# innnky/vispeech

Hardware: AMD Instinct MI355X
Metric: 44.1kHz samples/sec (higher is better)
Workload: dtype f32 (split-f16 MFMA, 3-term); 1 GPU; C3: 64 mixed zh/ja utterances (~5 s each) per GPU, 44.1 kHz, hop 512, phoneme/duration/F0/energy/noise supplied, random-init (synthetic) weights of configs/config.json; 2 batches in flight per GPU; utterances_per_gpu=64, global_batch=64, padded_frames=489, frames_padded=31296, frames_computed=28902, parallelism=shard1, generator=f16s, controls=all, batches_in_flight=2

## Files before the change

### vispeech_amd/csrc/conv_mfma.hip

```cpp
#include "kernels.h"

#include <cstdio>
#include <cstdlib>
#include <cstring>
#include <type_traits>

namespace vsp {

typedef float f32x16 __attribute__((ext_vector_type(16)));

size_t packed_conv_floats(int M, int Cin, int K) {
  const size_t mt = (M + 31) / 32, nc = (Cin + CONV_CK - 1) / CONV_CK;
  return mt * nc * (size_t)K * 1024;
}

void pack_conv_weights(float* dst, int M, int Cin, int K, const float* dense) {
  const int nc = (Cin + CONV_CK - 1) / CONV_CK;
  std::memset(dst, 0, packed_conv_floats(M, Cin, K) * sizeof(float));
  for (int row = 0; row < M; ++row) {
    const int mtile = row >> 5, rin = row & 31;
    for (int ci = 0; ci < Cin; ++ci) {
      const int chunk = ci / CONV_CK, cc = ci % CONV_CK;
      const int kk = cc >> 1, hh = cc & 1, lane = rin + 32 * hh, kg = kk >> 2, i = kk & 3;
      for (int tap = 0; tap < K; ++tap) {
        const size_t idx =
            (((((size_t)mtile * nc + chunk) * K + tap) * (CONV_CK / 8) + kg) * 64 + lane) * 4 + i;
        dst[idx] = dense[((size_t)row * Cin + ci) * K + tap];
      }
    }
  }
}

void pack_conv_weights_f16s(float* dst_f, int M, int Cin, int K, const float* dense) {
  const int nc = (Cin + CONV_CK - 1) / CONV_CK;
  std::memset(dst_f, 0, packed_conv_floats(M, Cin, K) * sizeof(float));
  uint16_t* dst = reinterpret_cast<uint16_t*>(dst_f);
  for (int row = 0; row < M; ++row) {
    const int mtile = row >> 5, rin = row & 31;
    for (int ci = 0; ci < Cin; ++ci) {
      const int chunk = ci / CONV_CK, cc = ci % CONV_CK;
      const int ks = cc >> 4, hh = (cc >> 3) & 1, j = cc & 7, lane = rin + 32 * hh;
      for (int tap = 0; tap < K; ++tap) {
        const float w = dense[((size_t)row * Cin + ci) * K + tap] * G16_WSCALE;
        const _Float16 h = (_Float16)w;
        const _Float16 l = (_Float16)(w - (float)h);
        const size_t blk = (((size_t)mtile * nc + chunk) * K + tap) * 2048;
        std::memcpy(dst + blk + ((size_t)(ks * 2 + 0) * 64 + lane) * 8 + j, &h, 2);
        std::memcpy(dst + blk + ((size_t)(ks * 2 + 1) * 64 + lane) * 8 + j, &l, 2);
      }
    }
  }
}

typedef _Float16 f16x8 __attribute__((ext_vector_type(8)));
typedef _Float16 f16x2 __attribute__((ext_vector_type(2)));
typedef unsigned u32x4 __attribute__((ext_vector_type(4)));

#ifndef CONV_DIAG
#define CONV_DIAG 0
#endif
#if CONV_DIAG & 1
#define CONV_MFMA16(a, b, c) ([&]() { asm volatile("" ::"v"(a), "v"(b)); return c; }())
#else
#define CONV_MFMA16(a, b, c) __builtin_amdgcn_mfma_f32_32x32x16_f16(a, b, c, 0, 0, 0)
#endif
#define CONV_RAW_BARRIER() asm volatile("s_waitcnt lgkmcnt(0)\n\ts_barrier" ::: "memory")
template <int N>
__device__ __forceinline__ void conv_vmcnt() {
  asm volatile("s_waitcnt vmcnt(%0)" ::"n"(N) : "memory");
}
constexpr int conv_ring_slots(int MT, int WM) { return 3; }

template <int MT, int NT>
struct ConvEpi {
  float bv[MT][16], cv[MT][16];
  unsigned rv[MT][NT][16], pv[MT][NT][16];
};
constexpr int CONV_OOR = 0x7ffffff0;

template <int MT, int NT, bool HOIST = true>
__device__ __forceinline__ void conv_epi_load(const ConvArgs& a, ConvEpi<MT, NT>& e, int mtile0, int n_mtiles, int t0, int wn,
                                              int l31, int h, int b, int what = 3) {
  const float* resb = a.res ? a.res + (size_t)b * a.r_bs : nullptr;
  float* outb = a.out + (size_t)b * a.o_bs;
  const float* condb = a.cond ? a.cond + (size_t)b * a.cond_bs : nullptr;
  const __amdgpu_buffer_rsrc_t ro = __builtin_amdgcn_make_buffer_rsrc(outb, 0, CONV_OOR, 0x00020000);
  const __amdgpu_buffer_rsrc_t rr = __builtin_amdgcn_make_buffer_rsrc(const_cast<float*>(resb ? resb : outb), 0, CONV_OOR, 0x00020000);
  const __amdgpu_buffer_rsrc_t ro2 = __builtin_amdgcn_make_buffer_rsrc(
      a.split_row ? a.out2 + (size_t)b * a.o2_bs : outb, 0, CONV_OOR, 0x00020000);
  auto row_vec = [&](const float* p, int row0, float* v) {
    v[0] = v[1] = v[2] = v[3] = 0.f;
    if (!p) return;
    if (row0 + 3 < a.M && (reinterpret_cast<uintptr_t>(p + row0) & 15) == 0) {
      const float4 t = *reinterpret_cast<const float4*>(p + row0);
      v[0] = t.x; v[1] = t.y; v[2] = t.z; v[3] = t.w;
    } else {
#pragma unroll
      for (int i = 0; i < 4; ++i)
        if (row0 + i < a.M) v[i] = p[row0 + i];
    }
  };
  const bool gate_ep = a.act == 2;
#pragma unroll
  for (int mt = 0; mt < MT; ++mt) {
    const int mtile = mtile0 + mt;
    if (what & 1) {
#pragma unroll
      for (int g = 0; g < 4; ++g) {
        row_vec(a.bias, mtile * 32 + 8 * g + 4 * h, &e.bv[mt][4 * g]);
        row_vec(condb, mtile * 32 + 8 * g + 4 * h, &e.cv[mt][4 * g]);
      }
    }
    if (!(what & 2)) continue;
    const bool second = a.split_row && mtile * 32 >= a.split_row;
    if constexpr (!HOIST) {
#pragma unroll
      for (int nt = 0; nt < NT; ++nt) {
        const int q = t0 + (wn * NT + nt) * 32 + l31;
        const bool qin = q < a.Nq && !gate_ep && mtile < n_mtiles;
#pragma unroll
        for (int r = 0; r < 16; ++r) {
          const int row = mtile * 32 + 8 * (r >> 2) + 4 * h + (r & 3);
          const bool st = qin && row < a.M;
          const int oo = st ? (row * (int)a.o_cs + q) * 4 : CONV_OOR;
// ... 309 lines not shown
    }
  }
  float v[16];
#pragma unroll
  for (int r = 0; r < 16; ++r) v[r] = tanhf(va[r]) * (1.f / (1.f + expf(-vb[r])));
  if (a.mask_post && !valid) {
#pragma unroll
    for (int r = 0; r < 16; ++r) v[r] = 0.f;
  }
#pragma unroll
  for (int r = 0; r < 16; ++r)
    __builtin_amdgcn_raw_buffer_store_b32(__float_as_uint(v[r]), ro, vo, (8 * (r >> 2) + (r & 3)) * ocs4, 0);
}

template <int S, int MT, int NT>
__device__ __forceinline__ void conv_store_slices(const ConvArgs& a, f32x16 (&acc)[MT][NT], int mtile0, int n_mtiles, int t0,
                                                  int wn, int l31, int h, int b, int len) {
#pragma unroll
  for (int ms = 0; ms < MT / S; ++ms)
#pragma unroll
    for (int nt = 0; nt < NT; ++nt) {
      const int tq = t0 + (wn * NT + nt) * 32;
      if constexpr (S == 1) {
        const int mtile = mtile0 + ms;
        if (mtile < n_mtiles && conv_tile_lean_ok(a, mtile)) {
          conv_tile_lean(a, acc[ms][nt], mtile, tq, l31, h, b, len);
          continue;
        }
      } else if constexpr (S == 2) {
        const int mtile = mtile0 + 2 * ms;
        if (conv_gate_lean_ok(a, mtile, n_mtiles)) {
          conv_gate_lean(a, acc[2 * ms][nt], acc[2 * ms + 1][nt], mtile, tq, l31, h, b, len);
          continue;
        }
      }
      f32x16 t[S][1];
#pragma unroll
      for (int u = 0; u < S; ++u) t[u][0] = acc[S * ms + u][nt];
      ConvEpi<S, 1> e;
      conv_epi_load<S, 1, false>(a, e, mtile0 + S * ms, n_mtiles, tq, 0, l31, h, b);
      conv_epi_store<S, 1>(a, t, e, mtile0 + S * ms, n_mtiles, tq, 0, l31, h, b, len);
    }
}
template <int MT, int NT>
__device__ __forceinline__ void conv_store_plain(const ConvArgs& a, f32x16 (&acc)[MT][NT], int mtile0, int n_mtiles, int t0,
                                                 int wn, int l31, int h, int b, int len) {
  if (a.act == 2) {
    if constexpr (MT % 2 == 0) conv_store_slices<2, MT, NT>(a, acc, mtile0, n_mtiles, t0, wn, l31, h, b, len);
  } else {
    conv_store_slices<1, MT, NT>(a, acc, mtile0, n_mtiles, t0, wn, l31, h, b, len);
  }
}

template <int MT, int NT, int WM, int WN, bool F16S, bool RING = false, bool PRUNE = false>
__global__ void __launch_bounds__(64 * WM * WN, F16S ? 2 : 1) conv1d_f32_mfma(ConvArgs a) {
  static_assert(!RING || F16S, "the weight ring serves the split-f16 path");
  static_assert(!PRUNE || (F16S && RING), "the pruned form is the split-f16 ring kernel");
  constexpr int BN = 32 * NT * WN;
  constexpr int LWP = BN + CONV_HALO;
  constexpr int NW = WM * WN;
  constexpr int KG = CONV_CK / 8;
  extern __shared__ __attribute__((aligned(16))) float xs[];
  constexpr int SB = MT * WM * 4096;
  constexpr int NS = conv_ring_slots(MT, WM), DEPTH = NS - 1;
  constexpr int PW = MT * WM * 4 / NW;
  static_assert(!RING || (MT * WM * 4) % NW == 0, "pieces divide over the waves");
  [[maybe_unused]] char* const ring = reinterpret_cast<char*>(xs) + (size_t)CONV_CK * LWP * sizeof(float);

  const int tid = threadIdx.x;
  const int wave = __builtin_amdgcn_readfirstlane(tid >> 6);
  const int lane = tid & 63;
  const int l31 = lane & 31, h = lane >> 5;
  const int wm = wave / WN, wn = wave % WN;
  const int b = blockIdx.z;
  const int t0 = blockIdx.x * BN;
  const int mtile0 = (blockIdx.y * WM + wm) * MT;
  const int n_mtiles = (a.M + 31) >> 5;
  const int len = a.lengths ? (int)a.lengths[b] : 0x7fffffff;
  const int LW = BN + (a.K - 1) * a.dil;
  const int total_it = a.nchunks * a.K;

  f32x16 acc[MT][NT];
#pragma unroll
  for (int mt = 0; mt < MT; ++mt)
#pragma unroll
    for (int nt = 0; nt < NT; ++nt)
#pragma unroll
      for (int r = 0; r < 16; ++r) {
        acc[mt][nt][r] = 0.f;
      }
  unsigned* const ph = reinterpret_cast<unsigned*>(xs);
  unsigned* const pl = ph + (CONV_CK / 2) * LWP;
  auto split_pair = [&](float x0, float x1, unsigned& whi, unsigned& wlo) { vsp_split_pair(x0, x1, whi, wlo); };

  const float4* wp4 = reinterpret_cast<const float4*>(a.wp);
  float4 a_cur[MT][KG], a_nxt[MT][KG];
  auto load_a = [&](int it, float4(&dst)[MT][KG]) {
#pragma unroll
    for (int mt = 0; mt < MT; ++mt) {
      const int mtile = mtile0 + mt;
      if (mtile < n_mtiles) {
        const float4* p = wp4 + (((size_t)mtile * total_it + it) * KG) * 64 + lane;
#pragma unroll
        for (int kg = 0; kg < KG; ++kg) dst[mt][kg] = p[kg * 64];
      } else {
#pragma unroll
        for (int kg = 0; kg < KG; ++kg) dst[mt][kg] = make_float4(0.f, 0.f, 0.f, 0.f);
      }
    }
  };
  if constexpr (!RING) load_a(0, a_cur);
  [[maybe_unused]] auto ring_dma = [&](int step) {
    char* dst = ring + (step % NS) * SB;
    if constexpr ((CONV_DIAG & 8) != 0) return;
#pragma unroll
    for (int u = 0; u < PW; ++u) {
      const int p = u * NW + wave;
      int mtile = blockIdx.y * (WM * MT) + (p >> 2);
      mtile = mtile < n_mtiles ? mtile : n_mtiles - 1;
      const float4* src = wp4 + (((size_t)mtile * total_it + step) * KG + (p & 3)) * 64 + lane;
      __builtin_amdgcn_global_load_lds((const __attribute__((address_space(1))) void*)src,
                                       (__attribute__((address_space(3))) void*)(dst + p * 1024), 16, 0, 0);
    }
  };
  constexpr bool PREF = RING && ((BN + CONV_HALO + 3) >> 2) <= 64;
  constexpr int RWPF = PREF ? (CONV_CK / 2) / NW : 1;
  constexpr int NPF = 2 * RWPF;
  [[maybe_unused]] int pf_step = -1000;
  [[maybe_unused]] auto ring_wait = [&](int step) {
    const int younger = total_it - 1 - step < DEPTH - 1 ? total_it - 1 - step : DEPTH - 1;
    const bool pf = PREF && step > pf_step && step - pf_step <= DEPTH;
    if (pf) {
      if (younger <= 0) conv_vmcnt<NPF>();
      else if (younger == 1) conv_vmcnt<PW + NPF>();
      else conv_vmcnt<2 * PW + NPF>();
    } else {
      if (younger <= 0) conv_vmcnt<0>();
      else if (younger == 1) conv_vmcnt<PW>();
      else conv_vmcnt<2 * PW>();
    }
  };
  static_assert(DEPTH <= 3, "ring_wait covers up to two younger steps");
  if constexpr (RING) {
#pragma unroll
    for (int d = 0; d < DEPTH; ++d)
      if (d < total_it) ring_dma(d);
  }

  const float* xb = a.x + (size_t)b * a.x_bs;
  const bool vec = ((a.x_cs & 3) == 0) && ((a.x_bs & 3) == 0) && ((reinterpret_cast<uintptr_t>(a.x) & 15) == 0);
  const int t_start = vec ? (((t0 - a.pad) >> 2) << 2) : (t0 - a.pad);
  const int off = (t0 - a.pad) - t_start;
  const int LW4 = (LW + off + 3) >> 2;
  const float* xsb = xs + h * LWP + wn * (NT * 32) + l31 + off;
  [[maybe_unused]] float4 pva[RWPF], pvb[RWPF];
  [[maybe_unused]] auto st_load = [&](int chunk) {
    const int t4 = t_start + 4 * lane;
    const bool tin = lane < LW4 && t4 >= 0 && t4 < a.T_in;
#pragma unroll
    for (int j = 0; j < RWPF; ++j) {
      const int ci = chunk * CONV_CK + 2 * (wave + j * NW);
      const float* pa = xb + (size_t)(tin && ci < a.Cin ? ci : 0) * a.x_cs + (tin ? t4 : 0);
      const float* pb = xb + (size_t)(tin && ci + 1 < a.Cin ? ci + 1 : 0) * a.x_cs + (tin ? t4 : 0);
      pva[j] = *reinterpret_cast<const float4*>(pa);
      pvb[j] = *reinterpret_cast<const float4*>(pb);
    }
  };
  typedef float f32x2v __attribute__((ext_vector_type(2)));
  [[maybe_unused]] const float slope_eff = a.in_act ? a.in_slope : 1.f;
  [[maybe_unused]] auto st_write = [&](int chunk) {
    if (lane >= LW4) return;
    const int t4 = t_start + 4 * lane;
    const bool tin = t4 >= 0 && t4 < a.T_in;
    const int lim = a.in_mask ? (len < a.T_in ? len : a.T_in) : a.T_in;
    const bool tfull = tin && t4 + 3 < lim;
#pragma unroll
    for (int j = 0; j < RWPF; ++j) {
      const int ci = chunk * CONV_CK + 2 * (wave + j * NW);
      const bool ina = tin && ci < a.Cin, inb = tin && ci + 1 < a.Cin;
      const float ea[4] = {pva[j].x, pva[j].y, pva[j].z, pva[j].w}, eb[4] = {pvb[j].x, pvb[j].y, pvb[j].z, pvb[j].w};
      unsigned wh4[4], wl4[4];
#pragma unroll
      for (int u = 0; u < 4; ++u) {
        f32x2v x = {ea[u], eb[u]};
        if (!(tfull && inb)) {
          x.x = (ina && t4 + u < lim) ? x.x : 0.f;
          x.y = (inb && t4 + u < lim) ? x.y : 0.f;
        }
        const f32x2v y = x * slope_eff;
        asm("v_max_f32 %0, %1, %2" : "=v"(x.x) : "v"(x.x), "v"(y.x));
        asm("v_max_f32 %0, %1, %2" : "=v"(x.y) : "v"(x.y), "v"(y.y));
        vsp_split_pair(x.x, x.y, wh4[u], wl4[u]);
      }
      const int o = (wave + j * NW) * LWP + 4 * lane;
      *reinterpret_cast<u32x4*>(ph + o) = u32x4{wh4[0], wh4[1], wh4[2], wh4[3]};
      *reinterpret_cast<u32x4*>(pl + o) = u32x4{wl4[0], wl4[1], wl4[2], wl4[3]};
    }
  };
  static_assert(!PRUNE || PREF, "the pruned form stages its window through the prefetch path");
  const bool pref = PRUNE || (PREF && vec && (CONV_DIAG & 2) == 0 && slope_eff >= 0.f && slope_eff <= 1.f);
  if constexpr (PREF) { if (pref) st_load(0); }
  int it = 0;
  for (int chunk = 0; chunk < a.nchunks; ++chunk) {
    if (pref) {
      if constexpr (PREF) st_write(chunk);
    } else if constexpr (PRUNE) {
    } else if (vec && F16S) {
      constexpr int RWP = (CONV_CK / 2) / NW;
      for (int q0 = 0; q0 < LW4; q0 += 64) {
        const int q4 = q0 + lane;
        const int t4 = t_start + 4 * q4;
        const bool tin = q4 < LW4 && t4 >= 0 && t4 < a.T_in;
        float4 va[RWP], vb[RWP];
#pragma unroll
        for (int j = 0; j < RWP; ++j) {
          const int ci = chunk * CONV_CK + 2 * (wave + j * NW);
          va[j] = vb[j] = make_float4(0.f, 0.f, 0.f, 0.f);
          if (tin && ci < a.Cin && !(CONV_DIAG & 2)) va[j] = *reinterpret_cast<const float4*>(xb + (size_t)ci * a.x_cs + t4);
          if (tin && ci + 1 < a.Cin && !(CONV_DIAG & 2)) vb[j] = *reinterpret_cast<const float4*>(xb + (size_t)(ci + 1) * a.x_cs + t4);
        }
        if (q4 < LW4) {
          const int lim = a.in_mask ? (len < a.T_in ? len : a.T_in) : a.T_in;
#pragma unroll
          for (int j = 0; j < RWP; ++j) {
            float ea[4] = {va[j].x, va[j].y, va[j].z, va[j].w}, eb[4] = {vb[j].x, vb[j].y, vb[j].z, vb[j].w};
            unsigned wh4[4], wl4[4];
#pragma unroll
            for (int u = 0; u < 4; ++u) {
              float x0 = (t4 + u < lim) ? ea[u] : 0.f, x1 = (t4 + u < lim) ? eb[u] : 0.f;
              if (a.in_act) { x0 = x0 > 0.f ? x0 : x0 * a.in_slope; x1 = x1 > 0.f ? x1 : x1 * a.in_slope; }
              split_pair(x0, x1, wh4[u], wl4[u]);
            }
            const int o = (wave + j * NW) * LWP + 4 * q4;
            *reinterpret_cast<u32x4*>(ph + o) = u32x4{wh4[0], wh4[1], wh4[2], wh4[3]};
            *reinterpret_cast<u32x4*>(pl + o) = u32x4{wl4[0], wl4[1], wl4[2], wl4[3]};
          }
        }
      }
    } else if (F16S) {
      for (int cp = wave; cp < CONV_CK / 2; cp += NW) {
        const int ci = chunk * CONV_CK + 2 * cp;
        const float* xr0 = xb + (size_t)ci * a.x_cs;
        const float* xr1 = xr0 + a.x_cs;
        for (int col = lane; col < LW; col += 64) {
          const int t = t0 - a.pad + col;
          float x0 = 0.f, x1 = 0.f;
          if (t >= 0 && t < a.T_in && !(a.in_mask && t >= len)) {
            if (ci < a.Cin) x0 = xr0[t];
            if (ci + 1 < a.Cin) x1 = xr1[t];
            if (a.in_act) { x0 = x0 > 0.f ? x0 : x0 * a.in_slope; x1 = x1 > 0.f ? x1 : x1 * a.in_slope; }
          }
          unsigned wh1, wl1;
          split_pair(x0, x1, wh1, wl1);
          ph[cp * LWP + col] = wh1;
          pl[cp * LWP + col] = wl1;
        }
      }
    } else if (vec) {
      constexpr int RW = CONV_CK / NW;
      for (int q0 = 0; q0 < LW4; q0 += 64) {
        const int q4 = q0 + lane;
        const int t4 = t_start + 4 * q4;
        const bool tin = q4 < LW4 && t4 >= 0 && t4 < a.T_in;
        float4 v[RW];
#pragma unroll
        for (int j = 0; j < RW; ++j) {
          const int ci = chunk * CONV_CK + wave + j * NW;
          v[j] = make_float4(0.f, 0.f, 0.f, 0.f);
          if (tin && ci < a.Cin) v[j] = *reinterpret_cast<const float4*>(xb + (size_t)ci * a.x_cs + t4);
        }
        if (q4 < LW4) {
          const int lim = a.in_mask ? (len < a.T_in ? len : a.T_in) : a.T_in;
#pragma unroll
          for (int j = 0; j < RW; ++j) {
            float e[4] = {v[j].x, v[j].y, v[j].z, v[j].w};
#pragma unroll
            for (int u = 0; u < 4; ++u) {
              float x = (t4 + u < lim) ? e[u] : 0.f;
              if (a.in_act) x = x > 0.f ? x : x * a.in_slope;
              e[u] = x;
            }
            *reinterpret_cast<float4*>(xs + (wave + j * NW) * LWP + 4 * q4) = make_float4(e[0], e[1], e[2], e[3]);
          }
        }
      }
    } else {
      for (int c = wave; c < CONV_CK; c += NW) {
        const int ci = chunk * CONV_CK + c;
        const bool cvalid = ci < a.Cin;
        const float* xr = xb + (size_t)ci * a.x_cs;
        float* dst = xs + c * LWP;
        for (int col = lane; col < LW; col += 64) {
          const int t = t0 - a.pad + col;
          float v = 0.f;
          if (cvalid && t >= 0 && t < a.T_in) {
            v = xr[t];
            if (a.in_mask && t >= len) v = 0.f;
            if (a.in_act) v = v > 0.f ? v : v * a.in_slope;
          }
          dst[col] = v;
        }
      }
    }
    if constexpr (!RING) __syncthreads();
    for (int tap = 0; tap < a.K; ++tap, ++it) {
      if constexpr (RING) {
        ring_wait(it);
        CONV_RAW_BARRIER();
        if (it + DEPTH < total_it) ring_dma(it + DEPTH);
        if constexpr (PREF) {
          if (pref && tap == 0 && chunk + 1 < a.nchunks) { st_load(chunk + 1); pf_step = it; }
        }
      } else {
        if (it + 1 < total_it) load_a(it + 1, a_nxt);
      }
      if constexpr (F16S) {
        const int col = wn * (NT * 32) + l31 + off + tap * a.dil;
#pragma unroll
        for (int ks = 0; ks < 2; ++ks) {
          f16x8 bh[NT], bl[NT];
#pragma unroll
          for (int nt = 0; nt < NT; ++nt) {
            const unsigned* p = ph + (8 * ks + 4 * h) * LWP + col + nt * 32;
            const unsigned* q = pl + (8 * ks + 4 * h) * LWP + col + nt * 32;
            bh[nt] = __builtin_bit_cast(f16x8, u32x4{p[0], p[LWP], p[2 * LWP], p[3 * LWP]});
            bl[nt] = __builtin_bit_cast(f16x8, u32x4{q[0], q[LWP], q[2 * LWP], q[3 * LWP]});
          }
#pragma unroll
          for (int mt = 0; mt < MT; ++mt) {
            f16x8 ah, al;
            if constexpr (RING) {
              const char* pa = ring + (it % NS) * SB + (wm * MT + mt) * 4096 + ks * 2048 + lane * 16;
              ah = *reinterpret_cast<const f16x8*>(pa);
              al = *reinterpret_cast<const f16x8*>(pa + 1024);
            } else {
              ah = __builtin_bit_cast(f16x8, a_cur[mt][2 * ks]);
              al = __builtin_bit_cast(f16x8, a_cur[mt][2 * ks + 1]);
            }
#pragma unroll
            for (int nt = 0; nt < NT; ++nt) acc[mt][nt] = CONV_MFMA16(ah, bh[nt], acc[mt][nt]);
#pragma unroll
            for (int nt = 0; nt < NT; ++nt) acc[mt][nt] = CONV_MFMA16(ah, bl[nt], acc[mt][nt]);
#pragma unroll
            for (int nt = 0; nt < NT; ++nt) acc[mt][nt] = CONV_MFMA16(al, bh[nt], acc[mt][nt]);
          }
        }
      }
      const float* xt = xsb + tap * a.dil;
#pragma unroll
      for (int kg = 0; kg < (F16S ? 0 : KG); ++kg) {
#pragma unroll
        for (int i = 0; i < 4; ++i) {
          const int kk = kg * 4 + i;
          float bv[NT];
#pragma unroll
          for (int nt = 0; nt < NT; ++nt) bv[nt] = xt[(2 * kk) * LWP + nt * 32];
#pragma unroll
          for (int mt = 0; mt < MT; ++mt) {
            const float av = i == 0 ? a_cur[mt][kg].x : i == 1 ? a_cur[mt][kg].y : i == 2 ? a_cur[mt][kg].z
                                                                                         : a_cur[mt][kg].w;
#pragma unroll
            for (int nt = 0; nt < NT; ++nt)
              acc[mt][nt] = __builtin_amdgcn_mfma_f32_32x32x2f32(av, bv[nt], acc[mt][nt], 0, 0, 0);
          }
        }
      }
      if constexpr (!RING) {
#pragma unroll
        for (int mt = 0; mt < MT; ++mt)
#pragma unroll
          for (int kg = 0; kg < KG; ++kg) a_cur[mt][kg] = a_nxt[mt][kg];
      }
    }
    if constexpr (RING) CONV_RAW_BARRIER();
    else __syncthreads();
  }

  if constexpr (F16S) {
#pragma unroll
    for (int mt = 0; mt < MT; ++mt)
#pragma unroll
      for (int nt = 0; nt < NT; ++nt)
#pragma unroll
        for (int r = 0; r < 16; ++r) acc[mt][nt][r] *= G16_UNSCALE;
  }
  if constexpr ((CONV_DIAG & 4) != 0) {
    float keep = 0.f;
#pragma unroll
    for (int mt = 0; mt < MT; ++mt)
#pragma unroll
      for (int nt = 0; nt < NT; ++nt) keep += acc[mt][nt][0];
    if (keep == 1.2345e-30f) a.out[0] = keep;
    return;
  }
  const float* resb = a.res ? a.res + (size_t)b * a.r_bs : nullptr;
  float* outb = a.out + (size_t)b * a.o_bs;
  const float* condb = a.cond ? a.cond + (size_t)b * a.cond_bs : nullptr;
  if (PRUNE || a.ups_s == 0) {
    conv_store_plain<MT, NT>(a, acc, mtile0, n_mtiles, t0, wn, l31, h, b, len);
    return;
  }
  if (a.act == 2) {
    if constexpr (MT % 2 == 0) {
#pragma unroll
      for (int mp = 0; mp < MT / 2; ++mp) {
        const int mtile = mtile0 + 2 * mp;
        if (mtile + 1 >= n_mtiles) continue;
#pragma unroll
        for (int nt = 0; nt < NT; ++nt) {
          const int q = t0 + (wn * NT + nt) * 32 + l31;
          if (q >= a.Nq) continue;
          const bool valid = q < len;
#pragma unroll
          for (int r = 0; r < 16; ++r) {
            const int rin = (r & 3) + 8 * (r >> 2) + 4 * h;
            const int ra = mtile * 32 + rin, rb = ra + 32;
            float va = acc[2 * mp][nt][r], vb = acc[2 * mp + 1][nt][r];
            if (a.bias) { va += a.bias[ra]; vb += a.bias[rb]; }
// ... 359 lines not shown
  }
#pragma unroll
  for (int mt = 0; mt < MT; ++mt)
#pragma unroll
    for (int nt = 0; nt < NT; ++nt)
#pragma unroll
      for (int r = 0; r < 16; ++r) acc[mt][nt][r] *= G16_UNSCALE;
  FR_STAMPT(30);
  conv_epi_store<MT, NT>(a, acc, epi, mtile0, n_mtiles, t0, wn, l31, h, b, len);
#ifdef FR_STAMPS
  FR_STAMPT(31);
  asm volatile("s_waitcnt vmcnt(0)" ::: "memory");
  FR_STAMPT(32);
#endif
}

#ifdef FR_STAMPS
static int g_fr_launch_no = 0;
static const int g_fr_on_vals[2] = {0, 1};
#endif
template <int MT, int NT, int WM, int WN, int K, int G, int RI, int WI>
static hipError_t launch_frame(const ConvArgs& a, int B, hipStream_t s) {
  constexpr int BN = 32 * NT * WN, BM = 32 * MT * WM, NW = WM * WN;
  constexpr int NF4 = CONV_CK * ((BN + (K == 1 ? 0 : FR_HALO)) / 4);
  constexpr size_t lds = (size_t)WI * G * ((NF4 + 64 * NW - 1) / (64 * NW)) * NW * 1024 + (size_t)RI * G * K * MT * WM * 4096;
  static_assert(lds <= 160 * 1024, "LDS budget");
  static std::atomic<uint64_t> attr_done{0};
  auto kern = conv_frame_f16s<MT, NT, WM, WN, K, G, RI, WI>;
  if (hipError_t e = set_max_dynamic_lds(reinterpret_cast<const void*>(kern), (int)lds, attr_done); e != hipSuccess) return e;
  dim3 grid((a.Nq + BN - 1) / BN, (a.M + BM - 1) / BM, B);
#ifdef FR_STAMPS
  {
    static int target = -2;
    if (target == -2) { const char* e = getenv("VSP_STAMP_FRAME"); target = e ? atoi(e) : -1; }
    const int on = g_fr_launch_no++ == target ? 1 : 0;
    (void)hipMemcpyToSymbolAsync(HIP_SYMBOL(g_fr_stamp_on), &g_fr_on_vals[on], sizeof(int), 0, hipMemcpyHostToDevice, s);
    if (on) fprintf(stderr, "[stamps] conv_frame_f16s<%d,%d,%d,%d,K%d,G%d,%d,%d> M %d Cin %d Nq %d grid %u x %u x %u\n", MT, NT, WM, WN, K,
                    G, RI, WI, a.M, a.Cin, a.Nq, grid.x, grid.y, grid.z);
  }
#endif
  hipLaunchKernelGGL(kern, grid, dim3(64 * WM * WN), lds, s, a);
  return hipGetLastError();
}
template <int MT, int NT, int WM, int WN>
static bool launch_frame_k(const ConvArgs& a, int B, hipStream_t s, hipError_t& e) {
  switch (a.K) {
    case 1: e = launch_frame<MT, NT, WM, WN, 1, 2, 3, 3>(a, B, s); return true;
    case 3: e = launch_frame<MT, NT, WM, WN, 3, 1, 3, 3>(a, B, s); return true;
    case 5: e = launch_frame<MT, NT, WM, WN, 5, 1, 2, 3>(a, B, s); return true;
    default: return false;
  }
}

template <int MT, int NT, int WM, int WN, bool F16S = false, bool RING = false, bool PRUNE = false>
static hipError_t launch_tile(const ConvArgs& a, int B, hipStream_t s) {
  constexpr int BN = 32 * NT * WN, BM = 32 * MT * WM;
  constexpr size_t lds = (size_t)CONV_CK * (BN + CONV_HALO) * sizeof(float) +
                         (RING ? (size_t)conv_ring_slots(MT, WM) * MT * WM * 4096 : 0);
  static_assert(lds <= 160 * 1024, "LDS budget (<= 80 KiB: two blocks per CU)");
  static std::atomic<uint64_t> attr_done{0};
  auto kern = conv1d_f32_mfma<MT, NT, WM, WN, F16S, RING, PRUNE>;
  if (hipError_t e = set_max_dynamic_lds(reinterpret_cast<const void*>(kern), (int)lds, attr_done); e != hipSuccess) return e;
  dim3 grid((a.Nq + BN - 1) / BN, (a.M + BM - 1) / BM, B);
  hipLaunchKernelGGL(kern, grid, dim3(64 * WM * WN), lds, s, a);
  return hipGetLastError();
}

template <int K, bool GATE>
__global__ void __launch_bounds__(256, 1) conv_frame_splitk(ConvArgs a) {
  constexpr int MT = 2, NT = 1, NWV = 4;
  constexpr int HALO = K == 1 ? 0 : FR_HALO;
  constexpr int BN = 32 * NT, LWP = BN + HALO, LWP4 = LWP / 4;
  constexpr int WBUF = CONV_CK * LWP * 4;
  constexpr int NIT = (16 * LWP4 + 63) / 64;
  constexpr int GT = 2;
  constexpr int GPC = (K + GT - 1) / GT;
  extern __shared__ __attribute__((aligned(16))) float xs[];
  char* const wbase = reinterpret_cast<char*>(xs);

  const int tid = threadIdx.x;
  const int wave = __builtin_amdgcn_readfirstlane(tid >> 6);
  const int lane = tid & 63;
  const int l31 = lane & 31, h = lane >> 5;
  const int b = blockIdx.z;
  const int t0 = blockIdx.x * BN;
  const int mtile0 = blockIdx.y * MT;
  const int n_mtiles = (a.M + 31) >> 5;
  const int nch = a.nchunks;
  const int total_it = nch * K;
  constexpr int FM = GATE ? 2 : 1;
  ConvEpi<FM, 1> epi;
  const bool finisher = wave < (GATE ? 1 : 2);
  const int fmt0 = mtile0 + (GATE ? 0 : wave);
  if (finisher) conv_epi_load<FM, 1>(a, epi, fmt0, n_mtiles, t0, 0, l31, h, b, 1);

  typedef float f32x4v __attribute__((ext_vector_type(4)));
  struct WSet { f32x4v w[GT][MT][4]; };
  const f32x4v* wp4 = reinterpret_cast<const f32x4v*>(a.wp);
  int mt_c[MT];
#pragma unroll
  for (int mt = 0; mt < MT; ++mt) mt_c[mt] = mtile0 + mt < n_mtiles ? mtile0 + mt : n_mtiles - 1;
  auto wload = [&](WSet& W, int c, int g) {
    c = c < nch ? c : nch - 1;
#pragma unroll
    for (int u = 0; u < GT; ++u) {
      int tap = g * GT + u;
      tap = tap < K ? tap : K - 1;
#pragma unroll
      for (int mt = 0; mt < MT; ++mt)
#pragma unroll
        for (int q = 0; q < 4; ++q)
          W.w[u][mt][q] = wp4[(((size_t)mt_c[mt] * total_it + c * K + tap) * 4 + q) * 64 + lane];
    }
  };
// ... 277 lines not shown
    }
    if (a.M <= 32 && !gate) {
      if (a.Nq >= 1024) return form_tile(1, 4, 1, 4, true, true);
      return form_tile(1, 1, 1, 2, true, true);
    }
    if (a.Nq <= 96) return form_tile(2, 1, 1, 2, true, true);
#ifdef VSP_EXPERIMENTS
    static int force_rows = -1;
    if (force_rows < 0) { const char* e = getenv("VSP_FRAME_TILE"); force_rows = e ? atoi(e) : 0; }
#else
    constexpr int force_rows = 0;
#endif
    const bool wide = force_rows ? force_rows == 128 : a.Nq >= 1024;
    const bool vec_ok = ((a.x_cs & 3) == 0) && ((a.x_bs & 3) == 0) && ((reinterpret_cast<uintptr_t>(a.x) & 15) == 0);
    const float sl_eff = a.in_act ? a.in_slope : 1.f;
    const bool prune_ok = vec_ok && sl_eff >= 0.f && sl_eff <= 1.f && a.ups_s == 0 && !(CONV_DIAG & 2);
    if (a.M <= 64 || (a.M % 128 != 0 && a.M < 256) || !wide) {
      if (a.Nq >= 1024) return form_tile(2, 2, 1, 4, true, true);
      if (prune_ok) return form_tile(2, 1, 1, 4, true, true, true);
      return form_tile(2, 1, 1, 4, true, true);
    }
    if (prune_ok) return form_tile(2, 2, 2, 2, true, true, true);
    return form_tile(2, 2, 2, 2, true, true);
  }
  if (a.f16s) {
    if (a.ups_s > 0) return form_of(VSP_CONV_FORM_NONE);
    if (a.M <= 32 && !gate) {
      if (a.Nq >= 1024) return form_tile(1, 4, 1, 4, true);
      return form_tile(1, 1, 1, 2, true);
    }
    if (a.Nq <= 96) return form_tile(2, 1, 1, 2, true);
    if (a.M <= 64 || (a.M % 128 != 0 && a.M < 256)) {
      if (a.Nq >= 1024) return form_tile(2, 2, 1, 4, true);
      return form_tile(2, 1, 1, 4, true);
    }
    return form_tile(2, 2, 2, 2, true);
  }
  if (a.M <= 32 && !gate) {
    if (a.Nq >= 1024) return form_tile(1, 4, 1, 4);
    return form_tile(1, 1, 1, 2);
  }
  if (a.Nq <= 96) return form_tile(2, 1, 1, 2);
  if (a.M <= 64 || (a.M % 128 != 0 && a.M < 256)) {
    if (a.Nq >= 1024) return form_tile(2, 4, 1, 4);
    return form_tile(2, 1, 1, 4);
  }
  return form_tile(2, 2, 2, 2);
}

static hipError_t launch_tile_form(const ConvForm& f, const ConvArgs& a, int B, hipStream_t s) {
  const int shape = f.mt * 1000 + f.nt * 100 + f.wm * 10 + f.wn;
  if (f.prune) {
    switch (shape) {
      case 2114: return launch_tile<2, 1, 1, 4, true, true, true>(a, B, s);
      case 2222: return launch_tile<2, 2, 2, 2, true, true, true>(a, B, s);
    }
  } else if (f.ring) {
    switch (shape) {
      case 1414: return launch_tile<1, 4, 1, 4, true, true>(a, B, s);
      case 1112: return launch_tile<1, 1, 1, 2, true, true>(a, B, s);
      case 2112: return launch_tile<2, 1, 1, 2, true, true>(a, B, s);
      case 2214: return launch_tile<2, 2, 1, 4, true, true>(a, B, s);
      case 2114: return launch_tile<2, 1, 1, 4, true, true>(a, B, s);
      case 2222: return launch_tile<2, 2, 2, 2, true, true>(a, B, s);
    }
  } else if (f.f16s) {
    switch (shape) {
      case 1414: return launch_tile<1, 4, 1, 4, true>(a, B, s);
      case 1112: return launch_tile<1, 1, 1, 2, true>(a, B, s);
      case 2112: return launch_tile<2, 1, 1, 2, true>(a, B, s);
      case 2214: return launch_tile<2, 2, 1, 4, true>(a, B, s);
      case 2114: return launch_tile<2, 1, 1, 4, true>(a, B, s);
      case 2222: return launch_tile<2, 2, 2, 2, true>(a, B, s);
    }
  } else {
    switch (shape) {
      case 1414: return launch_tile<1, 4, 1, 4>(a, B, s);
      case 1112: return launch_tile<1, 1, 1, 2>(a, B, s);
      case 2112: return launch_tile<2, 1, 1, 2>(a, B, s);
      case 2414: return launch_tile<2, 4, 1, 4>(a, B, s);
      case 2114: return launch_tile<2, 1, 1, 4>(a, B, s);
      case 2222: return launch_tile<2, 2, 2, 2>(a, B, s);
    }
  }
  return hipErrorInvalidValue;
}

hipError_t launch_conv(const ConvArgs& a, int B, hipStream_t s) {
  const ConvForm f = conv_form(a, B);
  hipError_t e = hipErrorInvalidValue;
  switch (f.kernel) {
    case VSP_CONV_FORM_COLS: return launch_conv_cols(a, B, s);
    case VSP_CONV_FORM_GEMV:
      hipLaunchKernelGGL(conv_t1_gemv, dim3((a.M + 31) / 32, B), dim3(256), 0, s, a);
      return hipGetLastError();
    case VSP_CONV_FORM_SPLITK:
      switch (f.k) {
        case 1: return launch_splitk<1>(a, B, s);
        case 3: return launch_splitk<3>(a, B, s);
        case 5: return launch_splitk<5>(a, B, s);
      }
      return e;
    case VSP_CONV_FORM_FRAME_SHORT: (void)launch_frame_k<2, 1, 1, 2>(a, B, s, e); return e;
    case VSP_CONV_FORM_FRAME: (void)launch_frame_k<2, 1, 1, 4>(a, B, s, e); return e;
    case VSP_CONV_FORM_TILE: return launch_tile_form(f, a, B, s);
    default: return e;
  }
}
// ... 3 lines not shown
```

Before: 210.2 million samples/s.

## Repack split-f16 input window into channel-octet planes and add multi-tap ring steps

Changes the LDS staging layout of the split-f16 input window from per-channel-pair rows to planes of 8-channel u32x4 groups with an odd-ish pitch. B-operand fragments then load as single 16-byte LDS reads instead of four strided 4-byte reads, and the staging stores are meant to avoid bank conflicts. Staging is redistributed so every thread loads 8 channels of one float4 column, and the next-chunk weight DMA is deferred until after the window is written. A TPS (taps per ring step) template parameter is added, but it defaults to 1, which adds complexity and vmcnt bookkeeping risk.

```diff
diff --git a/vispeech_amd/csrc/conv_mfma.hip b/vispeech_amd/csrc/conv_mfma.hip
--- a/vispeech_amd/csrc/conv_mfma.hip
+++ b/vispeech_amd/csrc/conv_mfma.hip
@@ -69,7 +69,12 @@
 __device__ __forceinline__ void conv_vmcnt() {
   asm volatile("s_waitcnt vmcnt(%0)" ::"n"(N) : "memory");
 }
-constexpr int conv_ring_slots(int MT, int WM) { return 3; }
+constexpr int conv_ring_slots(int MT, int WM, int TPS = 1) { return 3; }
+constexpr int CONV_TILE_TPS = 1;
+constexpr int conv_plane_pitch(int BN) { return BN + CONV_HALO + 1; }
+constexpr int conv_window_bytes(int BN, bool f16s) {
+  return f16s ? (2 * (CONV_CK / 8) * conv_plane_pitch(BN) * 16 + 1023) / 1024 * 1024 : CONV_CK * (BN + CONV_HALO) * (int)sizeof(float);
+}
 
 template <int MT, int NT>
 struct ConvEpi {
@@ -485,9 +490,10 @@
   }
 }
 
-template <int MT, int NT, int WM, int WN, bool F16S, bool RING = false, bool PRUNE = false>
+template <int MT, int NT, int WM, int WN, bool F16S, bool RING = false, bool PRUNE = false, int TPS = 1>
 __global__ void __launch_bounds__(64 * WM * WN, F16S ? 2 : 1) conv1d_f32_mfma(ConvArgs a) {
   static_assert(!RING || F16S, "the weight ring serves the split-f16 path");
+  static_assert(TPS >= 1 && (RING || TPS == 1), "multi-tap steps are ring steps");
   static_assert(!PRUNE || (F16S && RING), "the pruned form is the split-f16 ring kernel");
   constexpr int BN = 32 * NT * WN;
   constexpr int LWP = BN + CONV_HALO;
@@ -495,10 +501,13 @@
   constexpr int KG = CONV_CK / 8;
   extern __shared__ __attribute__((aligned(16))) float xs[];
   constexpr int SB = MT * WM * 4096;
-  constexpr int NS = conv_ring_slots(MT, WM), DEPTH = NS - 1;
+  constexpr int NS = conv_ring_slots(MT, WM, TPS), DEPTH = NS - 1;
   constexpr int PW = MT * WM * 4 / NW;
+  constexpr int PWS = TPS * PW;
   static_assert(!RING || (MT * WM * 4) % NW == 0, "pieces divide over the waves");
-  [[maybe_unused]] char* const ring = reinterpret_cast<char*>(xs) + (size_t)CONV_CK * LWP * sizeof(float);
+  constexpr int PP = conv_plane_pitch(BN);
+  static_assert(PP % 8 == 1 && LWP % 4 == 0, "plane pitch: conflict-free staging stores");
+  [[maybe_unused]] char* const ring = reinterpret_cast<char*>(xs) + conv_window_bytes(BN, F16S);
 
   const int tid = threadIdx.x;
   const int wave = __builtin_amdgcn_readfirstlane(tid >> 6);
@@ -512,6 +521,7 @@
   const int len = a.lengths ? (int)a.lengths[b] : 0x7fffffff;
   const int LW = BN + (a.K - 1) * a.dil;
   const int total_it = a.nchunks * a.K;
+  const int total_st = a.nchunks * ((a.K + TPS - 1) / TPS);
 
   f32x16 acc[MT][NT];
 #pragma unroll
@@ -522,8 +532,8 @@
       for (int r = 0; r < 16; ++r) {
         acc[mt][nt][r] = 0.f;
       }
-  unsigned* const ph = reinterpret_cast<unsigned*>(xs);
-  unsigned* const pl = ph + (CONV_CK / 2) * LWP;
+  u32x4* const ph = reinterpret_cast<u32x4*>(xs);
+  u32x4* const pl = ph + KG * PP;
   auto split_pair = [&](float x0, float x1, unsigned& whi, unsigned& wlo) { vsp_split_pair(x0, x1, whi, wlo); };
 
   const float4* wp4 = reinterpret_cast<const float4*>(a.wp);
@@ -543,41 +553,48 @@
     }
   };
   if constexpr (!RING) load_a(0, a_cur);
+  [[maybe_unused]] int dma_chunk = 0, dma_tap0 = 0;
   [[maybe_unused]] auto ring_dma = [&](int step) {
-    char* dst = ring + (step % NS) * SB;
+    char* dst = ring + (step % NS) * (TPS * SB);
     if constexpr ((CONV_DIAG & 8) != 0) return;
 #pragma unroll
-    for (int u = 0; u < PW; ++u) {
-      const int p = u * NW + wave;
-      int mtile = blockIdx.y * (WM * MT) + (p >> 2);
-      mtile = mtile < n_mtiles ? mtile : n_mtiles - 1;
-      const float4* src = wp4 + (((size_t)mtile * total_it + step) * KG + (p & 3)) * 64 + lane;
-      __builtin_amdgcn_global_load_lds((const __attribute__((address_space(1))) void*)src,
-                                       (__attribute__((address_space(3))) void*)(dst + p * 1024), 16, 0, 0);
-    }
+    for (int tt = 0; tt < TPS; ++tt) {
+      const int tap = dma_tap0 + tt < a.K ? dma_tap0 + tt : a.K - 1;
+      const int src_it = dma_chunk * a.K + tap;
+#pragma unroll
+      for (int u = 0; u < PW; ++u) {
+        const int p = u * NW + wave;
+        int mtile = blockIdx.y * (WM * MT) + (p >> 2);
+        mtile = mtile < n_mtiles ? mtile : n_mtiles - 1;
+        const float4* src = wp4 + (((size_t)mtile * total_it + src_it) * KG + (p & 3)) * 64 + lane;
+        __builtin_amdgcn_global_load_lds((const __attribute__((address_space(1))) void*)src,
+                                         (__attribute__((address_space(3))) void*)(dst + tt * SB + p * 1024), 16, 0, 0);
+      }
+    }
+    dma_tap0 += TPS;
+    if (dma_tap0 >= a.K) { dma_tap0 = 0; ++dma_chunk; }
   };
-  constexpr bool PREF = RING && ((BN + CONV_HALO + 3) >> 2) <= 64;
-  constexpr int RWPF = PREF ? (CONV_CK / 2) / NW : 1;
-  constexpr int NPF = 2 * RWPF;
+  constexpr bool PREF = RING && LWP <= 64 * NW;
+  constexpr int NPF = 8;
   [[maybe_unused]] int pf_step = -1000;
   [[maybe_unused]] auto ring_wait = [&](int step) {
-    const int younger = total_it - 1 - step < DEPTH - 1 ? total_it - 1 - step : DEPTH - 1;
+    const int younger = total_st - 1 - step < DEPTH - 1 ? total_st - 1 - step : DEPTH - 1;
     const bool pf = PREF && step > pf_step && step - pf_step <= DEPTH;
     if (pf) {
       if (younger <= 0) conv_vmcnt<NPF>();
-      else if (younger == 1) conv_vmcnt<PW + NPF>();
-      else conv_vmcnt<2 * PW + NPF>();
+      else if (younger == 1) conv_vmcnt<PWS + NPF>();
+      else conv_vmcnt<2 * PWS + NPF>();
     } else {
       if (younger <= 0) conv_vmcnt<0>();
-      else if (younger == 1) conv_vmcnt<PW>();
-      else conv_vmcnt<2 * PW>();
+      else if (younger == 1) conv_vmcnt<PWS>();
+      else conv_vmcnt<2 * PWS>();
     }
   };
-  static_assert(DEPTH <= 3, "ring_wait covers up to two younger steps");
+  static_assert(DEPTH >= 1 && DEPTH <= 3 && 2 * PWS + NPF < 64, "ring_wait covers up to two younger steps; vmcnt is six bits");
   if constexpr (RING) {
 #pragma unroll
     for (int d = 0; d < DEPTH; ++d)
-      if (d < total_it) ring_dma(d);
+      if (d < total_st) ring_dma(d);
   }
 
   const float* xb = a.x + (size_t)b * a.x_bs;
@@ -586,89 +603,78 @@
   const int off = (t0 - a.pad) - t_start;
   const int LW4 = (LW + off + 3) >> 2;
   const float* xsb = xs + h * LWP + wn * (NT * 32) + l31 + off;
-  [[maybe_unused]] float4 pva[RWPF], pvb[RWPF];
+  [[maybe_unused]] float4 pv[8];
   [[maybe_unused]] auto st_load = [&](int chunk) {
-    const int t4 = t_start + 4 * lane;
-    const bool tin = lane < LW4 && t4 >= 0 && t4 < a.T_in;
-#pragma unroll
-    for (int j = 0; j < RWPF; ++j) {
-      const int ci = chunk * CONV_CK + 2 * (wave + j * NW);
-      const float* pa = xb + (size_t)(tin && ci < a.Cin ? ci : 0) * a.x_cs + (tin ? t4 : 0);
-      const float* pb = xb + (size_t)(tin && ci + 1 < a.Cin ? ci + 1 : 0) * a.x_cs + (tin ? t4 : 0);
-      pva[j] = *reinterpret_cast<const float4*>(pa);
-      pvb[j] = *reinterpret_cast<const float4*>(pb);
-    }
+    const int g = tid >> 2, c0 = chunk * CONV_CK + 8 * (tid & 3);
+    const int t4 = t_start + 4 * g;
+    const bool tin = g < LW4 && t4 >= 0 && t4 < a.T_in;
+#pragma unroll
+    for (int i = 0; i < 8; ++i)
+      pv[i] = *reinterpret_cast<const float4*>(xb + (size_t)(tin && c0 + i < a.Cin ? c0 + i : 0) * a.x_cs + (tin ? t4 : 0));
   };
-  typedef float f32x2v __attribute__((ext_vector_type(2)));
   [[maybe_unused]] const float slope_eff = a.in_act ? a.in_slope : 1.f;
-  [[maybe_unused]] auto st_write = [&](int chunk) {
-    if (lane >= LW4) return;
-    const int t4 = t_start + 4 * lane;
+  [[maybe_unused]] auto st_convert = [&](int chunk, int pos, const auto& v, auto maxf) {
+    const int g = pos >> 2, plane = pos & 3;
+    if (g >= LW4) return;
+    const int t4 = t_start + 4 * g, c0 = chunk * CONV_CK + 8 * plane;
     const bool tin = t4 >= 0 && t4 < a.T_in;
     const int lim = a.in_mask ? (len < a.T_in ? len : a.T_in) : a.T_in;
-    const bool tfull = tin && t4 + 3 < lim;
-#pragma unroll
-    for (int j = 0; j < RWPF; ++j) {
-      const int ci = chunk * CONV_CK + 2 * (wave + j * NW);
-      const bool ina = tin && ci < a.Cin, inb = tin && ci + 1 < a.Cin;
-      const float ea[4] = {pva[j].x, pva[j].y, pva[j].z, pva[j].w}, eb[4] = {pvb[j].x, pvb[j].y, pvb[j].z, pvb[j].w};
-      unsigned wh4[4], wl4[4];
-#pragma unroll
-      for (int u = 0; u < 4; ++u) {
-        f32x2v x = {ea[u], eb[u]};
-        if (!(tfull && inb)) {
-          x.x = (ina && t4 + u < lim) ? x.x : 0.f;
-          x.y = (inb && t4 + u < lim) ? x.y : 0.f;
-        }
-        const f32x2v y = x * slope_eff;
-        asm("v_max_f32 %0, %1, %2" : "=v"(x.x) : "v"(x.x), "v"(y.x));
-        asm("v_max_f32 %0, %1, %2" : "=v"(x.y) : "v"(x.y), "v"(y.y));
-        vsp_split_pair(x.x, x.y, wh4[u], wl4[u]);
-      }
-      const int o = (wave + j * NW) * LWP + 4 * lane;
-      *reinterpret_cast<u32x4*>(ph + o) = u32x4{wh4[0], wh4[1], wh4[2], wh4[3]};
-      *reinterpret_cast<u32x4*>(pl + o) = u32x4{wl4[0], wl4[1], wl4[2], wl4[3]};
-    }
+    const bool full = tin && t4 + 3 < lim && c0 + 7 < a.Cin;
+    u32x4* const dh = ph + plane * PP + 4 * g;
+    u32x4* const dl = pl + plane * PP + 4 * g;
+#pragma unroll
+    for (int u = 0; u < 4; ++u) {
+      float e[8];
+#pragma unroll
+      for (int i = 0; i < 8; ++i) e[i] = u == 0 ? v[i].x : u == 1 ? v[i].y : u == 2 ? v[i].z : v[i].w;
+      if (!full) {
+#pragma unroll
+        for (int i = 0; i < 8; ++i) e[i] = (tin && c0 + i < a.Cin && t4 + u < lim) ? e[i] : 0.f;
+      }
+#pragma unroll
+      for (int i = 0; i < 8; ++i) {
+        if constexpr (decltype(maxf)::value) {
+          const float y = e[i] * slope_eff;
+          asm("v_max_f32 %0, %1, %2" : "=v"(e[i]) : "v"(e[i]), "v"(y));
+        } else {
+          if (a.in_act) e[i] = e[i] > 0.f ? e[i] : e[i] * a.in_slope;
+        }
+      }
+      unsigned wh[4], wl[4];
+#pragma unroll
+      for (int j = 0; j < 4; ++j) vsp_split_pair(e[2 * j], e[2 * j + 1], wh[j], wl[j]);
+      dh[u] = u32x4{wh[0], wh[1], wh[2], wh[3]};
+      dl[u] = u32x4{wl[0], wl[1], wl[2], wl[3]};
+    }
+  };
+  [[maybe_unused]] auto st_write = [&](int chunk) {
+    asm volatile("" ::"v"(pv[7].w));
+    st_convert(chunk, tid, pv, std::true_type{});
   };
   static_assert(!PRUNE || PREF, "the pruned form stages its window through the prefetch path");
   const bool pref = PRUNE || (PREF && vec && (CONV_DIAG & 2) == 0 && slope_eff >= 0.f && slope_eff <= 1.f);
   if constexpr (PREF) { if (pref) st_load(0); }
   int it = 0;
+  [[maybe_unused]] bool dma_late = false;
   for (int chunk = 0; chunk < a.nchunks; ++chunk) {
     if (pref) {
-      if constexpr (PREF) st_write(chunk);
+      if constexpr (PREF) {
+        st_write(chunk);
+        if (dma_late) { ring_dma(it + DEPTH - 1); dma_late = false; }
+      }
     } else if constexpr (PRUNE) {
     } else if (vec && F16S) {
-      constexpr int RWP = (CONV_CK / 2) / NW;
-      for (int q0 = 0; q0 < LW4; q0 += 64) {
-        const int q4 = q0 + lane;
-        const int t4 = t_start + 4 * q4;
-        const bool tin = q4 < LW4 && t4 >= 0 && t4 < a.T_in;
-        float4 va[RWP], vb[RWP];
-#pragma unroll
-        for (int j = 0; j < RWP; ++j) {
-          const int ci = chunk * CONV_CK + 2 * (wave + j * NW);
-          va[j] = vb[j] = make_float4(0.f, 0.f, 0.f, 0.f);
-          if (tin && ci < a.Cin && !(CONV_DIAG & 2)) va[j] = *reinterpret_cast<const float4*>(xb + (size_t)ci * a.x_cs + t4);
-          if (tin && ci + 1 < a.Cin && !(CONV_DIAG & 2)) vb[j] = *reinterpret_cast<const float4*>(xb + (size_t)(ci + 1) * a.x_cs + t4);
-        }
-        if (q4 < LW4) {
-          const int lim = a.in_mask ? (len < a.T_in ? len : a.T_in) : a.T_in;
-#pragma unroll
-          for (int j = 0; j < RWP; ++j) {
-            float ea[4] = {va[j].x, va[j].y, va[j].z, va[j].w}, eb[4] = {vb[j].x, vb[j].y, vb[j].z, vb[j].w};
-            unsigned wh4[4], wl4[4];
-#pragma unroll
-            for (int u = 0; u < 4; ++u) {
-              float x0 = (t4 + u < lim) ? ea[u] : 0.f, x1 = (t4 + u < lim) ? eb[u] : 0.f;
-              if (a.in_act) { x0 = x0 > 0.f ? x0 : x0 * a.in_slope; x1 = x1 > 0.f ? x1 : x1 * a.in_slope; }
-              split_pair(x0, x1, wh4[u], wl4[u]);
-            }
-            const int o = (wave + j * NW) * LWP + 4 * q4;
-            *reinterpret_cast<u32x4*>(ph + o) = u32x4{wh4[0], wh4[1], wh4[2], wh4[3]};
-            *reinterpret_cast<u32x4*>(pl + o) = u32x4{wl4[0], wl4[1], wl4[2], wl4[3]};
-          }
-        }
+      for (int p0 = 0; p0 < 4 * LW4; p0 += 64 * NW) {
+        const int pos = p0 + tid, g = pos >> 2, c0 = chunk * CONV_CK + 8 * (pos & 3);
+        const int t4 = t_start + 4 * g;
+        const bool tin = g < LW4 && t4 >= 0 && t4 < a.T_in;
+        float4 v[8];
+#pragma unroll
+        for (int i = 0; i < 8; ++i) {
+          v[i] = make_float4(0.f, 0.f, 0.f, 0.f);
+          if (tin && c0 + i < a.Cin && !(CONV_DIAG & 2)) v[i] = *reinterpret_cast<const float4*>(xb + (size_t)(c0 + i) * a.x_cs + t4);
+        }
+        st_convert(chunk, pos, v, std::false_type{});
       }
     } else if (F16S) {
       for (int cp = wave; cp < CONV_CK / 2; cp += NW) {
@@ -685,8 +691,8 @@
           }
           unsigned wh1, wl1;
           split_pair(x0, x1, wh1, wl1);
-          ph[cp * LWP + col] = wh1;
-          pl[cp * LWP + col] = wl1;
+          reinterpret_cast<unsigned*>(ph + (cp >> 2) * PP + col)[cp & 3] = wh1;
+          reinterpret_cast<unsigned*>(pl + (cp >> 2) * PP + col)[cp & 3] = wl1;
         }
       }
     } else if (vec) {
@@ -736,17 +742,24 @@
       }
     }
     if constexpr (!RING) __syncthreads();
-    for (int tap = 0; tap < a.K; ++tap, ++it) {
+    for (int tap0 = 0; tap0 < a.K; tap0 += TPS, ++it) {
       if constexpr (RING) {
         ring_wait(it);
         CONV_RAW_BARRIER();
-        if (it + DEPTH < total_it) ring_dma(it + DEPTH);
+        if (it + DEPTH < total_st) {
+          if (PREF && pref && tap0 + TPS >= a.K && chunk + 1 < a.nchunks) dma_late = true;
+          else ring_dma(it + DEPTH);
+        }
         if constexpr (PREF) {
-          if (pref && tap == 0 && chunk + 1 < a.nchunks) { st_load(chunk + 1); pf_step = it; }
+          if (pref && tap0 == 0 && chunk + 1 < a.nchunks) { st_load(chunk + 1); pf_step = it; }
         }
       } else {
         if (it + 1 < total_it) load_a(it + 1, a_nxt);
       }
+#pragma unroll
+      for (int tt = 0; tt < TPS; ++tt) {
+      const int tap = tap0 + tt;
+      if (TPS > 1 && tap >= a.K) break;
       if constexpr (F16S) {
         const int col = wn * (NT * 32) + l31 + off + tap * a.dil;
 #pragma unroll
@@ -754,16 +767,14 @@
           f16x8 bh[NT], bl[NT];
 #pragma unroll
           for (int nt = 0; nt < NT; ++nt) {
-            const unsigned* p = ph + (8 * ks + 4 * h) * LWP + col + nt * 32;
-            const unsigned* q = pl + (8 * ks + 4 * h) * LWP + col + nt * 32;
-            bh[nt] = __builtin_bit_cast(f16x8, u32x4{p[0], p[LWP], p[2 * LWP], p[3 * LWP]});
-            bl[nt] = __builtin_bit_cast(f16x8, u32x4{q[0], q[LWP], q[2 * LWP], q[3 * LWP]});
+            bh[nt] = __builtin_bit_cast(f16x8, ph[(2 * ks + h) * PP + col + nt * 32]);
+            bl[nt] = __builtin_bit_cast(f16x8, pl[(2 * ks + h) * PP + col + nt * 32]);
           }
 #pragma unroll
           for (int mt = 0; mt < MT; ++mt) {
             f16x8 ah, al;
             if constexpr (RING) {
-              const char* pa = ring + (it % NS) * SB + (wm * MT + mt) * 4096 + ks * 2048 + lane * 16;
+              const char* pa = ring + (it % NS) * (TPS * SB) + tt * SB + (wm * MT + mt) * 4096 + ks * 2048 + lane * 16;
               ah = *reinterpret_cast<const f16x8*>(pa);
               al = *reinterpret_cast<const f16x8*>(pa + 1024);
             } else {
@@ -797,6 +808,7 @@
               acc[mt][nt] = __builtin_amdgcn_mfma_f32_32x32x2f32(av, bv[nt], acc[mt][nt], 0, 0, 0);
           }
         }
+      }
       }
       if constexpr (!RING) {
 #pragma unroll
@@ -1262,14 +1274,14 @@
   }
 }
 
-template <int MT, int NT, int WM, int WN, bool F16S = false, bool RING = false, bool PRUNE = false>
+template <int MT, int NT, int WM, int WN, bool F16S = false, bool RING = false, bool PRUNE = false, int TPS = 1>
 static hipError_t launch_tile(const ConvArgs& a, int B, hipStream_t s) {
   constexpr int BN = 32 * NT * WN, BM = 32 * MT * WM;
-  constexpr size_t lds = (size_t)CONV_CK * (BN + CONV_HALO) * sizeof(float) +
-                         (RING ? (size_t)conv_ring_slots(MT, WM) * MT * WM * 4096 : 0);
+  constexpr size_t lds = (size_t)conv_window_bytes(BN, F16S) +
+                         (RING ? (size_t)conv_ring_slots(MT, WM, TPS) * TPS * MT * WM * 4096 : 0);
   static_assert(lds <= 160 * 1024, "LDS budget (<= 80 KiB: two blocks per CU)");
   static std::atomic<uint64_t> attr_done{0};
-  auto kern = conv1d_f32_mfma<MT, NT, WM, WN, F16S, RING, PRUNE>;
+  auto kern = conv1d_f32_mfma<MT, NT, WM, WN, F16S, RING, PRUNE, TPS>;
   if (hipError_t e = set_max_dynamic_lds(reinterpret_cast<const void*>(kern), (int)lds, attr_done); e != hipSuccess) return e;
   dim3 grid((a.Nq + BN - 1) / BN, (a.M + BM - 1) / BM, B);
   hipLaunchKernelGGL(kern, grid, dim3(64 * WM * WN), lds, s, a);
@@ -1653,8 +1665,8 @@
   const int shape = f.mt * 1000 + f.nt * 100 + f.wm * 10 + f.wn;
   if (f.prune) {
     switch (shape) {
-      case 2114: return launch_tile<2, 1, 1, 4, true, true, true>(a, B, s);
-      case 2222: return launch_tile<2, 2, 2, 2, true, true, true>(a, B, s);
+      case 2114: return launch_tile<2, 1, 1, 4, true, true, true, CONV_TILE_TPS>(a, B, s);
+      case 2222: return launch_tile<2, 2, 2, 2, true, true, true, CONV_TILE_TPS>(a, B, s);
     }
   } else if (f.ring) {
     switch (shape) {
```

Result: no change. 210.2 million samples/s (-0.0%).
